# biodatageeks/polars-bio

Measured on AMD Instinct MI355X. Metric: overlap-pairs/sec, higher is better.
Workload: dtype int32; 1 GPU; overlap_100M_5M_24contig; probe_rows=100000000, build_rows=5000000, contigs=24, filter_op=Strict, parallelism=single GPU

## Files before the change

include/ivjoin.h:

```cpp
#ifndef IVJOIN_H
#define IVJOIN_H

#include <stdint.h>

#ifdef __cplusplus
extern "C" {
#endif

#define IVJ_OK            0
#define IVJ_EINVAL       -1
#define IVJ_EHIP         -2
#define IVJ_ENOMEM       -3
#define IVJ_ECAPACITY    -4
#define IVJ_ESTATE       -5
#define IVJ_EPEER        -6

#define IVJ_FILTER_WEAK   0
#define IVJ_FILTER_STRICT 1

#define IVJ_NEAREST_IGNORE_LEFT  1
#define IVJ_NEAREST_IGNORE_RIGHT 2

typedef struct ivj_ctx ivj_ctx;
typedef struct ivj_index ivj_index;
// ... 339 lines not shown
                                    const ivj_opts* opts, const char* suffix1, int64_t batch_rows, int64_t limit, void* out_stream);
int ivj_nearest_arrow_stream(ivj_ctx* ctx, void* df1_stream, void* df2_stream, const char* const* cols1, const char* const* cols2,
                             const ivj_opts* opts, const char* suffix1, const char* suffix2, int32_t with_distance, int64_t batch_rows,
                             int64_t limit, void* out_stream);

int ivj_overlap_arrow_stream_lazy(ivj_ctx* ctx, void* df1_stream, void* df2_stream, const char* const* cols1, const char* const* cols2,
                                  const ivj_opts* opts, const char* suffix1, const char* suffix2, int64_t batch_rows, int64_t max_batch_rows,
                                  int64_t limit, void* out_stream);
int ivj_count_overlaps_arrow_stream_lazy(ivj_ctx* ctx, void* df1_stream, void* df2_stream, const char* const* cols1, const char* const* cols2,
                                         const ivj_opts* opts, const char* suffix1, int64_t batch_rows, int64_t max_batch_rows, int64_t limit,
                                         void* out_stream);
int ivj_nearest_arrow_stream_lazy(ivj_ctx* ctx, void* df1_stream, void* df2_stream, const char* const* cols1, const char* const* cols2,
                                  const ivj_opts* opts, const char* suffix1, const char* suffix2, int32_t with_distance, int64_t batch_rows,
                                  int64_t max_batch_rows, int64_t limit, void* out_stream);

typedef struct {
    int64_t n1, n2;
    int32_t *contig1, *start1, *end1;
    int32_t *contig2, *start2, *end2;
    int32_t n_contigs;
    int64_t* name_offsets;
    char* name_bytes;
} ivj_arrow_keys;
int ivj_arrow_encode_keys(void* df1_stream, void* df2_stream, const char* const* cols1, const char* const* cols2, ivj_arrow_keys* out);
void ivj_arrow_keys_free(ivj_arrow_keys* keys);
int ivj_arrow_take_stream(void* in_stream, const int64_t* idx, int64_t n, int64_t batch_rows, void* out_stream);


int ivj_dev_alloc(ivj_ctx* ctx, int64_t bytes, void** out);
int ivj_dev_free(ivj_ctx* ctx, void* p);
int ivj_memcpy_h2d(ivj_ctx* ctx, void* dst_dev, const void* src_host, int64_t bytes);
int ivj_memcpy_d2h(ivj_ctx* ctx, void* dst_host, const void* src_dev, int64_t bytes);


int ivj_host_narrow_i32(const void* src, int32_t src_bytes, int32_t is_unsigned, int64_t n, int32_t* dst, int64_t* out_min, int64_t* out_max,
                        int32_t threads);

int ivj_host_encode_utf8(const void* offsets, int32_t offset_bytes, const uint8_t* data, const uint8_t* validity, int64_t validity_bit0, int64_t n,
                         int32_t* ids, int64_t* dict_rows, int32_t dict_cap, int32_t* n_values, int32_t threads);

int ivj_host_encode_keys64(const uint64_t* keys, int64_t n, int32_t* ids, int64_t* dict_rows, int32_t dict_cap, int32_t* n_values, int32_t threads);

int ivj_host_remap_i32(const void* idx, int32_t idx_bytes, int64_t n, const int32_t* remap, int64_t remap_len, int32_t* out, uint8_t* seen,
                       int32_t threads);

int ivj_host_take(const void* src, int32_t elem_bytes, int64_t n_src, const int32_t* idx, int64_t n, void* dst, int32_t threads);

int ivj_host_scatter(const void* src, int32_t row_bytes, int64_t n, const int32_t* idx, int64_t n_dst, void* dst, const int32_t* remap, int64_t remap_len,
                     int32_t threads);

int ivj_host_shard(const int32_t* contig, const int32_t* start, const int32_t* end, int64_t n, const int32_t* owner, int32_t n_contigs, int32_t world,
                   int64_t* counts, int32_t* const* out_contig, int32_t* const* out_start, int32_t* const* out_end, int32_t* const* out_row, int32_t threads);
int ivj_host_contig_hist(const int32_t* contig, int64_t n, int32_t n_contigs, int64_t* hist, int32_t threads);
int ivj_host_group_ids(const int32_t* probe_contig, const int32_t* const* probe_codes, int64_t n_probe, const int32_t* build_contig,
                       const int32_t* const* build_codes, int64_t n_build, int32_t n_cols, const int32_t* cards, int32_t n_contigs,
                       int32_t* probe_gid, int32_t* build_gid, int32_t* group_keys, int64_t keys_cap, int32_t* n_groups, int32_t threads);

int ivj_host_widen_i32(const int32_t* src, int64_t n, int64_t* dst, int32_t threads);

#ifdef __cplusplus
}
#endif
#endif
```

polars-bio_amd/csrc/host_index.hip.h:

```cpp
#pragma once

namespace {

int build_tables(ivj_ctx* ctx, ivj_index* ix);
bool cs_geom(int64_t n, int nc, int want_rows, CsGeom& g);
size_t cs_index_bytes(const CsGeom& g);
void cs_index_carve(ivj_index* ix, char* p);

int ensure_hier(ivj_ctx* ctx, ivj_index* ix) {
    if (ix->hier_built || ix->n <= 0) return IVJ_OK;
    const HierShape h = hier_shape(ix->n);
    const int64_t wgs = (((ix->n + 15) & ~(int64_t)15) + HIER_WG_ROWS - 1) / HIER_WG_ROWS;
    LAUNCH(ctx, "hier_low", k_hier_low, (unsigned)wgs, 256, (const int2*)ix->ep, ix->n, ix->hier, h);
    if (h.nlev >= 3) LAUNCH(ctx, "hier_high", k_hier_high, 1, 256, ix->hier, h, wgs);
    HIP_TRY(hipGetLastError());
    ix->hier_built = true;
    return IVJ_OK;
}

int need_tables(ivj_ctx* ctx, ivj_index* ix) {
    if (!ix->has_tables) return fail(IVJ_ESTATE, "this index was built for merge / cluster only (with_end_order & 2): it has no lookup tables");
    if (ix->tables_built) return IVJ_OK;
    return build_tables(ctx, ix);
}
// ... 216 lines not shown
    p.z_meta = align_up(sizeof(V3Meta)); p.z_st = align_up((size_t)V3_BUCKETS * 8); p.z_hs = align_up((size_t)p.hs_tiles * 8); p.z_tick = align_up(16);
    p.zero_bytes = p.z_meta + p.z_st + p.z_hs + p.z_tick;
    return p;
}
int index_sort_v3(ivj_ctx* ctx, ivj_index* ix, const ivj_side* build, const ivj_opts* opts, bool* done) {
    *done = false;
    const int64_t n = build->n;
    const int nc = opts->n_contigs;
    const int64_t tiles = (n + OS_TILE - 1) / OS_TILE;
    const V3Plan VP = v3_plan(n);
    const int64_t chunk = VP.chunk, hist_len = VP.hist_len, hs_tiles = VP.hs_tiles;
    const int nchunks = VP.nchunks;
    const size_t z_meta = VP.z_meta, z_st = VP.z_st, z_hs = VP.z_hs, zero_bytes = VP.zero_bytes;
    OsSort S;
    const size_t v2_bytes = os_sort_plan(S, n, nc);
    const bool own_z = ix->ix3_z == nullptr;
    IVJ_TRY(arena_reserve(ctx, std::max(v2_bytes, (own_z ? zero_bytes : 0) + align_up((size_t)hist_len * 4) + align_up((size_t)n * 16)) + 4096));
    char* z = own_z ? arena_take<char>(ctx, zero_bytes) : ix->ix3_z;
    uint32_t* hist = arena_take<uint32_t>(ctx, (size_t)hist_len);
    int4* recs = arena_take<int4>(ctx, (size_t)n);
    V3Meta* meta = (V3Meta*)z;
    unsigned long long* st_local = (unsigned long long*)(z + z_meta);
    unsigned long long* st_scan = (unsigned long long*)(z + z_meta + z_st);
    uint32_t* tick_scan = (uint32_t*)(z + z_meta + z_st + z_hs);
    if (own_z) HIP_TRY(hipMemsetAsync(z, 0, zero_bytes, ctx->stream));
    const size_t pass_lds = (size_t)v3_pass_lds().total;
    if (!ctx->ix3_attr_set) {
        HIP_TRY(hipFuncSetAttribute(reinterpret_cast<const void*>(&k_v3_scatter), hipFuncAttributeMaxDynamicSharedMemorySize, (int)pass_lds));
        HIP_TRY(hipFuncSetAttribute(reinterpret_cast<const void*>(&k_v3_local<true>), hipFuncAttributeMaxDynamicSharedMemorySize, 160 * 1024 - 256));
        HIP_TRY(hipFuncSetAttribute(reinterpret_cast<const void*>(&k_v3_local<false>), hipFuncAttributeMaxDynamicSharedMemorySize, 160 * 1024 - 256));
        ctx->ix3_attr_set = true;
    }
    const unsigned sgrid = (unsigned)(tiles < 512 ? tiles : 512);
    LAUNCH(ctx, "ix3_stats", k_v3_stats, sgrid, OS_THREADS, build->start, build->end, build->contig, n, nc, meta);
    LAUNCH(ctx, "ix3_hist", k_v3_hist, nchunks, OS_THREADS, build->contig, build->start, n, nc, meta, (int)chunk, nchunks, hist);
    LAUNCH(ctx, "ix_scan", (k_scan_lb_u32<SumOp, true>), hs_tiles, OS_THREADS, hist, hist_len, 0u, tick_scan, st_scan);
    const int ms_max = ctx->env_ix_merge >= 0 ? std::min(ctx->env_ix_merge, V3_MAX_MERGE) : V3_MAX_MERGE;
    const uint32_t hw_seq = ctx->hw ? ++ctx->hw_seq : 0u;
    LAUNCH(ctx, "ix3_check", k_v3_check, 1, OS_THREADS, (const uint32_t*)hist, nchunks, n, ms_max, meta, ctx->hw_dev, hw_seq);
    if (!ctx->hw) HIP_TRY(hipMemcpyAsync(ctx->h_total + 6, &meta->bad, 8, hipMemcpyDeviceToHost, ctx->stream));
    if (!ctx->ix3_event) HIP_TRY(hipEventCreateWithFlags(&ctx->ix3_event, hipEventDisableTiming));
    HIP_TRY(hipEventRecord(ctx->ix3_event, ctx->stream));
    t_begin(ctx, "ix3_pass");
    hipLaunchKernelGGL(k_v3_scatter, dim3((unsigned)nchunks), dim3(OS_THREADS), pass_lds, ctx->stream, build->contig, build->start, build->end, build->row_id,
                       recs, n, nc, meta, (int)chunk, nchunks, (const uint32_t*)hist);
    t_end(ctx);
    HIP_TRY(hipGetLastError());
    HIP_TRY(wait_event(ctx, ctx->ix3_event));
    uint32_t* hv = reinterpret_cast<uint32_t*>(ctx->h_total + 6);
    if (ctx->hw) {
        const volatile uint32_t* w = reinterpret_cast<volatile uint32_t*>(ctx->hw);
        if (w[2] == hw_seq) { hv[0] = w[0]; hv[1] = w[1]; }
        else {
            ++ctx->hw_misses;
            HIP_TRY(hipMemcpyAsync(ctx->h_total + 6, &meta->bad, 8, hipMemcpyDeviceToHost, ctx->stream));
            HIP_TRY(hipStreamSynchronize(ctx->stream));
        }
    }
    const uint32_t max_bucket = hv[1] & 0xffffffu;
    const int ms = (int)(hv[1] >> 24);
    if (hv[0] != 0u || max_bucket > (uint32_t)V3_CAP) { ++ctx->ix3_fallbacks; ++ctx->ix3_fallback_streak; ctx->ix3_builds_since_fallback = 0; return IVJ_OK; }
    ctx->ix3_fallback_streak = 0;
    const int cap = (int)std::max<uint32_t>(1024u, (max_bucket + 1023u) / 1024u * 1024u);
    const int bin_bits = cap <= 1024 ? 10 : (cap <= 2048 ? 11 : V3_MAX_BIN_BITS);
    const bool stage = ctx->env_ix_stage >= 0 ? ctx->env_ix_stage != 0 : cap <= 2048;
    const size_t local_lds = (size_t)v3_local_lds(cap, 1 << bin_bits, stage).total;
    with_bool(stage, [&](auto STAGE) {
        LAUNCH_LDS(ctx, "ix3_local", k_v3_local<STAGE>, V3_BUCKETS >> ms, OS_THREADS, local_lds, (const int4*)recs, (const uint32_t*)hist, nchunks, n, nc, cap, bin_bits, ms,
                   meta, st_local, ix->b_start, ix->ep, ix->b_row, ix->b_contig, ix->seg, ix->flags);
    });
    HIP_TRY(hipGetLastError());
    *done = true;
    return IVJ_OK;
}

int build_tables(ivj_ctx* ctx, ivj_index* ix) {
    const int nc = ix->n_contigs;
    const int64_t n = ix->n;
    if (n > 0 && nc > 0) {
        const int64_t lb_tiles = (ix->bins_len + LB_TILE - 1) / LB_TILE;
        const size_t zb = align_up((size_t)lb_tiles * 8) + align_up(16);
        IVJ_TRY(arena_reserve(ctx, zb + 4096));
        char* z = arena_take<char>(ctx, zb);
        HIP_TRY(hipMemsetAsync(z, 0, zb, ctx->stream));
        HIP_TRY(hipMemsetAsync(ix->bins, 0, (size_t)ix->bins_len * 4, ctx->stream));
        LAUNCH(ctx, "contig_meta", k_contig_meta, grid1d(nc, 256), 256, (const int32_t*)ix->seg, (const int32_t*)ix->b_start, nc, ix->cmeta);
        LAUNCH(ctx, "bins_mark", k_bins_mark, grid1d(n, 256), 256, (const int32_t*)ix->b_start, (const int32_t*)ix->b_contig, n, nc,
               (const int4*)ix->cmeta, ix->bins);
        LAUNCH(ctx, "bins_scan", (k_scan_lb_u32<MaxOp, false>), lb_tiles, OS_THREADS, ix->bins, ix->bins_len, 0u,
               (uint32_t*)(z + align_up((size_t)lb_tiles * 8)), (unsigned long long*)z);
        LAUNCH(ctx, "bins_records", k_bins_records, grid1d(ix->bins_len, 256), 256, (const uint32_t*)ix->bins, ix->bins_len,
// ... 95 lines not shown
```

polars-bio_amd/csrc/ivjoin.hip:

```cpp
#include "../../include/ivjoin.h"

#include <hip/hip_runtime.h>

#include <algorithm>
#include <atomic>
#include <chrono>
#include <cstdio>
#include <cstdlib>
#include <cstring>
#include <string>
#include <vector>
#include <thread>
#include <type_traits>

#include "probe.hip.h"
#include "slice.hip.h"
#include "cslice.hip.h"
#include "onesweep.hip.h"
#include "ixsort3.hip.h"
#include "scan.hip.h"
#include "group.hip.h"
#include "depth.hip.h"
#include "depth_sum.hip.h"
#include "depth_profile.hip.h"
// ... 1717 lines not shown
    *out = nullptr;
    if (bytes == 0) return IVJ_OK;
    hipError_t e = hipMalloc(out, (size_t)bytes);
    if (e != hipSuccess) return fail(IVJ_ENOMEM, std::string("hipMalloc: ") + hipGetErrorString(e));
    return IVJ_OK;
} IVJ_ABI_CATCH
int ivj_dev_free(ivj_ctx* ctx, void* p) try {
    if (!ctx) return fail(IVJ_EINVAL, "ctx is NULL");
    if (!p) return IVJ_OK;
    DeviceGuard g(ctx->device);
    HIP_TRY(hipStreamSynchronize(ctx->stream));
    HIP_TRY(hipFree(p));
    return IVJ_OK;
} IVJ_ABI_CATCH
int ivj_memcpy_h2d(ivj_ctx* ctx, void* dst_dev, const void* src_host, int64_t bytes) try {
    if (!ctx || bytes < 0) return fail(IVJ_EINVAL, "bad argument");
    if (bytes == 0) return IVJ_OK;
    DeviceGuard g(ctx->device);
    HostXfer copy(ctx->stream, &ctx->xfer);
    copy.h2d(dst_dev, src_host, (size_t)bytes);
    HIP_TRY(copy.finish());
    return IVJ_OK;
} IVJ_ABI_CATCH
int ivj_memcpy_d2h(ivj_ctx* ctx, void* dst_host, const void* src_dev, int64_t bytes) try {
    if (!ctx || bytes < 0) return fail(IVJ_EINVAL, "bad argument");
    if (bytes == 0) return IVJ_OK;
    DeviceGuard g(ctx->device);
    HostXfer copy(ctx->stream, &ctx->xfer);
    copy.d2h(dst_host, src_dev, (size_t)bytes);
    HIP_TRY(copy.finish());
    return IVJ_OK;
} IVJ_ABI_CATCH

}

#include "host_frontdoor.hip.h"
#include "host_arrow_stream.hip.h"
```

polars-bio_amd/csrc/ixsort3.hip.h:

```cpp
#pragma once
#include "onesweep.hip.h"

namespace ivj {

constexpr int V3_BUCKETS = OS_RADIX;
constexpr int V3_ITEMS = 4;
constexpr int V3_CAP = OS_THREADS * V3_ITEMS;
constexpr int V3_MAX_KEYS = 256;
constexpr int V3_MAX_BIN_BITS = 12;

struct V3Meta {
    uint32_t inverted;
    uint32_t pad0;
    uint32_t bad;
    uint32_t max_bucket;
    uint32_t ticket;
    uint32_t wbits;
    uint32_t pad[2];
    unsigned long long M;
    unsigned long long span;
    uint32_t cmax[V3_MAX_KEYS];
    uint32_t cimn[V3_MAX_KEYS];
    uint32_t base[V3_MAX_KEYS];
};

__device__ __forceinline__ uint32_t v3_bucket(uint32_t lin, unsigned long long M) { return (uint32_t)(((unsigned long long)lin * M) >> 32); }

__device__ __forceinline__ void v3_load_tables(const V3Meta* __restrict__ meta, int nk, uint32_t* l_base, uint32_t* l_cmin) {
    for (int k = threadIdx.x; k < nk; k += OS_THREADS) { l_base[k] = meta->base[k]; l_cmin[k] = ~meta->cimn[k]; }
}

__global__ __launch_bounds__(OS_THREADS) void k_v3_stats(const int32_t* __restrict__ start, const int32_t* __restrict__ end,
                                                        const int32_t* __restrict__ contig, int64_t n, int32_t n_contigs, V3Meta* __restrict__ meta) {
    __shared__ uint32_t l_mx[V3_MAX_KEYS], l_imn[V3_MAX_KEYS];
    __shared__ uint32_t l_inv;
    const int tid = threadIdx.x, nk = n_contigs + 1;
    for (int k = tid; k < V3_MAX_KEYS; k += OS_THREADS) { l_mx[k] = 0u; l_imn[k] = 0u; }
    if (tid == 0) l_inv = 0u;
    __syncthreads();
    uint32_t inv = 0;
    for (int64_t i = (int64_t)blockIdx.x * OS_THREADS + tid; i < n; i += (int64_t)gridDim.x * OS_THREADS) {
        const int32_t s = start[i], c0 = contig[i];
        const int c = (uint32_t)c0 < (uint32_t)n_contigs ? c0 : n_contigs;
        const uint32_t u = flip(s);
        if (u > l_mx[c]) atomicMax(&l_mx[c], u);
        if (~u > l_imn[c]) atomicMax(&l_imn[c], ~u);
        if (s > end[i] && c < n_contigs) inv = 1u;
    }
    if (inv) l_inv = 1u;
    __syncthreads();
    for (int k = tid; k < nk; k += OS_THREADS) {
        const uint32_t a = l_mx[k], b = l_imn[k];
        if (a > os_ld(&meta->cmax[k])) atomicMax(&meta->cmax[k], a);
        if (b > os_ld(&meta->cimn[k])) atomicMax(&meta->cimn[k], b);
    }
    if (tid == 0 && l_inv && !os_ld(&meta->inverted)) atomicOr(&meta->inverted, 1u);
}

struct V3Geom { unsigned long long M; uint32_t wbits; bool bad; };
__device__ __forceinline__ V3Geom v3_geometry(V3Meta* __restrict__ meta, int nk, uint32_t* l_base, uint32_t* l_cmin, unsigned long long* l_ws , bool record) {
    const int tid = threadIdx.x;
    unsigned long long sp = 0;
    uint32_t cmn = 0xffffffffu;
    if (tid < nk) {
        const uint32_t cmx = meta->cmax[tid], cim = meta->cimn[tid];
        cmn = ~cim;
        if ((cmx | cim) != 0u) sp = (unsigned long long)(cmx - cmn) + 1ull;
    }
    unsigned long long total;
    const unsigned long long pre = sl_block_exclusive_sum<unsigned long long>(sp, l_ws, &total);
    if (tid < nk) { l_base[tid] = (uint32_t)pre; l_cmin[tid] = cmn; if (record) meta->base[tid] = (uint32_t)pre; }
    if (tid == 0) {
        const bool bad = total == 0ull || total > 0xffffffffull;
        const unsigned long long M = bad ? 1ull : (1ull << 43) / total;
        const unsigned long long wmax = (1ull << 32) / M;
        const uint32_t wbits = (uint32_t)os_bits_for(wmax > 0xffffffffull ? 0xffffffffu : (uint32_t)wmax);
        l_ws[OS_WAVES] = M;
        l_ws[OS_WAVES + 1] = (unsigned long long)wbits | (bad ? (1ull << 32) : 0ull);
        if (record) { meta->bad = bad ? 1u : 0u; meta->span = total; meta->M = M; meta->wbits = wbits; }
    }
    __syncthreads();
    V3Geom g;
    g.M = l_ws[OS_WAVES];
    g.wbits = (uint32_t)l_ws[OS_WAVES + 1];
    g.bad = (l_ws[OS_WAVES + 1] >> 32) != 0ull;
    return g;
}

__global__ __launch_bounds__(OS_THREADS) void k_v3_hist(const int32_t* __restrict__ contig, const int32_t* __restrict__ start, int64_t n,
                                                       int32_t n_contigs, V3Meta* __restrict__ meta, int chunk, int nchunks,
                                                       uint32_t* __restrict__ hist) {
    __shared__ uint32_t h[V3_BUCKETS];
    __shared__ uint32_t l_base[V3_MAX_KEYS], l_cmin[V3_MAX_KEYS];
    __shared__ unsigned long long l_ws[OS_WAVES + 2];
    const V3Geom g = v3_geometry(meta, n_contigs + 1, l_base, l_cmin, l_ws, blockIdx.x == 0);
    if (g.bad) return;
    const unsigned long long M = g.M;
    for (int k = threadIdx.x; k < V3_BUCKETS; k += OS_THREADS) h[k] = 0;
    __syncthreads();
    const int64_t base = (int64_t)blockIdx.x * chunk;
    const int64_t end = base + chunk < n ? base + chunk : n;
    for (int64_t i = base + threadIdx.x; i < end; i += OS_THREADS) {
        const int32_t c0 = contig[i];
        const int c = (uint32_t)c0 < (uint32_t)n_contigs ? c0 : n_contigs;
        const uint32_t lin = l_base[c] + (flip(start[i]) - l_cmin[c]);
        atomicAdd(&h[v3_bucket(lin, M)], 1u);
    }
    __syncthreads();
    for (int k = threadIdx.x; k < V3_BUCKETS; k += OS_THREADS) hist[(int64_t)k * nchunks + blockIdx.x] = h[k];
}

constexpr int V3_MAX_MERGE = 5;
__global__ __launch_bounds__(OS_THREADS) void k_v3_check(const uint32_t* __restrict__ off, int nchunks, int64_t n, int ms_max, V3Meta* __restrict__ meta,
                                                        uint32_t* __restrict__ hw, uint32_t hw_seq) {
    __shared__ uint32_t wmx[V3_MAX_MERGE + 1][OS_WAVES];
    if (meta->bad) {
        if (threadIdx.x == 0 && hw) { hw_store(hw + 0, 1u); hw_store(hw + 1, 0u); hw_store(hw + 2, hw_seq); }
        return;
    }
    const int tid = threadIdx.x;
    uint32_t sz[2];
#pragma unroll
    for (int q = 0; q < 2; ++q) {
        const int b = 2 * tid + q;
        const uint32_t a = off[(int64_t)b * nchunks];
        const uint32_t z = b + 1 < V3_BUCKETS ? off[(int64_t)(b + 1) * nchunks] : (uint32_t)n;
        sz[q] = z - a;
    }
    uint32_t mx[V3_MAX_MERGE + 1];
    mx[0] = sz[0] > sz[1] ? sz[0] : sz[1];
    uint32_t sum = sz[0] + sz[1];
    mx[1] = sum;
#pragma unroll
    for (int k = 2; k <= V3_MAX_MERGE; ++k) { sum += __shfl_xor(sum, 1 << (k - 2), kWave); mx[k] = sum; }
#pragma unroll
    for (int k = 0; k <= V3_MAX_MERGE; ++k) {
#pragma unroll
        for (int d = kWave / 2; d > 0; d >>= 1) { const uint32_t o = __shfl_xor(mx[k], d, kWave); mx[k] = o > mx[k] ? o : mx[k]; }
        if ((tid & (kWave - 1)) == 0) wmx[k][tid / kWave] = mx[k];
    }
    __syncthreads();
    if (tid == 0) {
        uint32_t best = 0, best_ms = 0;
#pragma unroll
        for (int k = 0; k <= V3_MAX_MERGE; ++k) {
            uint32_t m = 0;
#pragma unroll
            for (int w = 0; w < OS_WAVES; ++w) m = wmx[k][w] > m ? wmx[k][w] : m;
            if (k == 0 || (k <= ms_max && m <= (uint32_t)V3_CAP)) { best = m; best_ms = (uint32_t)k; }
        }
        meta->max_bucket = best | (best_ms << 24);
        if (hw) { hw_store(hw + 0, 0u); hw_store(hw + 1, best | (best_ms << 24)); hw_store(hw + 2, hw_seq); }
    }
}

struct V3PassLds { OsPassLds P; int tbase, tcmin, total; };
__host__ __device__ inline V3PassLds v3_pass_lds() {
    V3PassLds L;
    L.P = os_pass_lds();
    int o = (L.P.total + 15) & ~15;
    L.tbase = o; o += 4 * V3_MAX_KEYS;
    L.tcmin = o; o += 4 * V3_MAX_KEYS;
    L.total = o;
    return L;
}

__global__ __launch_bounds__(OS_THREADS) void k_v3_scatter(const int32_t* __restrict__ contig, const int32_t* __restrict__ start,
                                                          const int32_t* __restrict__ end, const int32_t* __restrict__ row_id,
                                                          int4* __restrict__ dst, int64_t n, int32_t n_contigs, V3Meta* __restrict__ meta,
                                                          int chunk, int nchunks, const uint32_t* __restrict__ off ) {
    extern __shared__ __attribute__((aligned(16))) unsigned char os_lds[];
    const V3PassLds LL = v3_pass_lds();
    const OsPassLds& L = LL.P;
    int4* l_rec = reinterpret_cast<int4*>(os_lds + L.rec);
    unsigned short* wcnt = reinterpret_cast<unsigned short*>(os_lds + L.wcnt);
    unsigned short* l_d = reinterpret_cast<unsigned short*>(os_lds + L.d);
    uint32_t* base = reinterpret_cast<uint32_t*>(os_lds + L.base);
    uint32_t* lstart = reinterpret_cast<uint32_t*>(os_lds + L.lstart);
    uint32_t* wsum = reinterpret_cast<uint32_t*>(os_lds + L.wsum);
    uint32_t* l_base = reinterpret_cast<uint32_t*>(os_lds + LL.tbase);
    uint32_t* l_cmin = reinterpret_cast<uint32_t*>(os_lds + LL.tcmin);
    if (meta->bad) return;
    const unsigned long long M = meta->M;
    const int tid = threadIdx.x, w = tid / kWave, lane = tid & (kWave - 1);
    v3_load_tables(meta, n_contigs + 1, l_base, l_cmin);
    for (int k = tid; k < OS_RADIX; k += OS_THREADS) base[k] = off[(int64_t)k * nchunks + blockIdx.x];
    for (int k = tid; k < OS_RADIX * OS_WAVES / 2; k += OS_THREADS) reinterpret_cast<uint32_t*>(wcnt)[k] = 0;
    __syncthreads();
    const int64_t cbase = (int64_t)blockIdx.x * chunk;
    const int64_t cend = cbase + chunk < n ? cbase + chunk : n;
    const uint64_t lt = lanemask_lt();
    unsigned short* my = wcnt + w * OS_RADIX;
    const int el0 = w * (OS_ITEMS * kWave) + lane;
    int4 nxt[OS_ITEMS];
    auto load_tile = [&](int64_t tb) {
        const int tn = (int)((cend - tb) < (int64_t)OS_TILE ? (cend - tb) : (int64_t)OS_TILE);
#pragma unroll
        for (int j = 0; j < OS_ITEMS; ++j) {
            const int il = el0 + j * kWave;
            nxt[j] = il < tn ? os_load_record(true, contig, start, end, row_id, nullptr, tb + il, n_contigs) : make_int4(0, 0, 0, 0);
        }
    };
    if (cbase < cend) load_tile(cbase);
    for (int64_t tbase = cbase; tbase < cend; tbase += OS_TILE) {
        const int tile_n = (int)((cend - tbase) < (int64_t)OS_TILE ? (cend - tbase) : (int64_t)OS_TILE);
        int4 r[OS_ITEMS];
        uint32_t d[OS_ITEMS], rank[OS_ITEMS];
#pragma unroll
        for (int j = 0; j < OS_ITEMS; ++j) {
            r[j] = nxt[j];
            d[j] = v3_bucket(l_base[r[j].w] + (flip(r[j].x) - l_cmin[r[j].w]), M);
        }
        if (tbase + OS_TILE < cend) load_tile(tbase + OS_TILE);
#pragma unroll
        for (int j = 0; j < OS_ITEMS; ++j) {
            const bool valid = el0 + j * kWave < tile_n;
            uint64_t peers = __ballot(valid);
#pragma unroll
            for (int b = 0; b < OS_BITS; ++b) {
                const bool bit = (d[j] >> b) & 1u;
                const uint64_t m = __ballot(valid && bit);
// ... 265 lines not shown
```

polars-bio_amd/polars_bio_amd/_engine.py:

```python
from __future__ import annotations

import ctypes as C
import os
import threading
from typing import Optional, Tuple

import numpy as np

_HERE = os.path.dirname(os.path.abspath(__file__))
LIB_PATH = os.path.join(_HERE, "lib", "libivjoin_hip.so")

FILTER_WEAK = 0
FILTER_STRICT = 1

ABI_SYMBOLS = [
    "ivj_last_error", "ivj_version", "ivj_abi_version", "ivj_device_count", "ivj_host_mem_available", "ivj_ctx_create", "ivj_ctx_destroy",
    "ivj_ctx_set_stream", "ivj_ctx_sync", "ivj_ctx_enable_timing", "ivj_ctx_get_timings", "ivj_ctx_profile_mark",
    "ivj_overlap", "ivj_pairs_free", "ivj_count_overlaps", "ivj_nearest",
    "ivj_index_build_dev", "ivj_index_free", "ivj_overlap_count_dev", "ivj_overlap_fill_dev", "ivj_overlap_fused_dev",
    "ivj_count_overlaps_dev", "ivj_nearest_dev",
    "ivj_overlap_thresh", "ivj_count_overlaps_thresh", "ivj_overlap_thresh_dev", "ivj_count_overlaps_thresh_dev",
    "ivj_overlap_select", "ivj_rowsel_free", "ivj_overlap_select_dev", "ivj_overlap_outer",
    "ivj_side_from_arrow", "ivj_materialize_dev", "ivj_overlap_fused_rows_dev", "ivj_take_dev", "ivj_take", "ivj_overlap_rows", "ivj_rows_free", "ivj_rows_export_arrow",
    "ivj_subtract", "ivj_complement", "ivj_pieces_free", "ivj_subtract_dev",
    "ivj_merge", "ivj_merged_free", "ivj_cluster", "ivj_coverage", "ivj_cluster_dev", "ivj_merge_dev", "ivj_coverage_dev",
    "ivj_merge_agg", "ivj_merge_agg_free", "ivj_merge_agg_dev",
    "ivj_overlap_agg", "ivj_overlap_agg_dev", "ivj_permute_overlaps", "ivj_permute_overlaps_dev",
    "ivj_overlap_wagg", "ivj_overlap_wagg_dev", "ivj_signal_profile", "ivj_signal_profile_dev",
    "ivj_overlap_bases", "ivj_overlap_bases_dev", "ivj_depth_profile", "ivj_depth_profile_dev",
    "ivj_depth", "ivj_blocks_free", "ivj_depth_dev", "ivj_depth_summary", "ivj_depth_summary_dev",
    "ivj_setop", "ivj_regions_free", "ivj_set_stats", "ivj_setop_dev", "ivj_set_stats_dev",
    "ivj_multi_inter", "ivj_segments_free", "ivj_multi_inter_dev",
    "ivj_stream_open", "ivj_stream_submit", "ivj_stream_flush", "ivj_stream_set_nearest_ignore", "ivj_stream_close",
    "ivj_dev_alloc", "ivj_dev_free", "ivj_memcpy_h2d", "ivj_memcpy_d2h",
    "ivj_comm_unique_id", "ivj_comm_create", "ivj_comm_create_local", "ivj_comm_destroy", "ivj_comm_info",
    "ivj_allgather_counts", "ivj_allgatherv_dev", "ivj_overlap_allgather_dev",
    "ivj_count_overlaps_allgather_dev", "ivj_nearest_allgather_dev",
    "ivj_overlap_arrow_stream", "ivj_count_overlaps_arrow_stream", "ivj_nearest_arrow_stream", "ivj_arrow_encode_keys", "ivj_arrow_keys_free",
    "ivj_overlap_arrow_stream_lazy", "ivj_count_overlaps_arrow_stream_lazy", "ivj_nearest_arrow_stream_lazy",
    "ivj_arrow_take_stream",
    "ivj_host_shard", "ivj_host_contig_hist", "ivj_group_ids_dev", "ivj_host_group_ids",
    "ivj_host_narrow_i32", "ivj_host_encode_utf8", "ivj_host_encode_keys64", "ivj_host_remap_i32", "ivj_host_take", "ivj_host_scatter", "ivj_host_widen_i32",
]

ABI_VERSION = 6
STREAM_OVERLAP, STREAM_COUNT, STREAM_NEAREST = 0, 1, 2
NEAREST_IGNORE_LEFT, NEAREST_IGNORE_RIGHT = 1, 2
DEPTH_PROFILE_MAX_BINS = 4096

SETOP_INTERSECTION, SETOP_UNION, SETOP_DIFFERENCE, SETOP_SYMMETRIC_DIFFERENCE = 0, 1, 2, 3
SETOPS = {"intersection": SETOP_INTERSECTION, "union": SETOP_UNION, "difference": SETOP_DIFFERENCE,
          "symmetric_difference": SETOP_SYMMETRIC_DIFFERENCE}

MAX_FRAMES = 64
MULTI_SEGMENTS, MULTI_CONSENSUS = 0, 1

AGG_SUM, AGG_MIN, AGG_MAX, AGG_MEAN, AGG_COUNT = 1, 2, 4, 8, 16
AGG_OPS = {"sum": AGG_SUM, "min": AGG_MIN, "max": AGG_MAX, "mean": AGG_MEAN, "count": AGG_COUNT}
AGG_I64, AGG_F64 = 0, 1
MAX_AGG_COLS = 16

ROW_COLUMNS = ("probe_idx", "build_idx", "contig", "start_1", "end_1", "start_2", "end_2")


IVJ_ECAPACITY, IVJ_ESTATE, IVJ_EPEER = -4, -5, -6

SELECT_SEMI, SELECT_ANTI = 0, 1
# ... 191 lines not shown
        L.ivj_permute_overlaps.argtypes = [vp, P, P, O, vp, vp, C.c_int64, vp, vp]
        L.ivj_permute_overlaps_dev.argtypes = [vp, vp, P, O, vp, vp, C.c_int64, vp, vp]
        L.ivj_depth.argtypes = [vp, P, O, C.POINTER(_Blocks)]
        L.ivj_blocks_free.argtypes = [C.POINTER(_Blocks)]
        L.ivj_blocks_free.restype = None
        L.ivj_depth_dev.argtypes = [vp, vp, O, C.c_int64, vp, vp, vp, vp, C.POINTER(C.c_int64)]
        L.ivj_setop.argtypes = [vp, P, P, O, C.c_int32, C.POINTER(_Regions)]
        L.ivj_regions_free.argtypes = [C.POINTER(_Regions)]
        L.ivj_regions_free.restype = None
        L.ivj_set_stats.argtypes = [vp, P, P, O, C.POINTER(C.c_int64), C.POINTER(C.c_int64)]
        L.ivj_setop_dev.argtypes = [vp, vp, vp, O, C.c_int32, C.c_int64, vp, vp, vp, C.POINTER(C.c_int64)]
        L.ivj_set_stats_dev.argtypes = [vp, vp, vp, O, C.POINTER(C.c_int64), C.POINTER(C.c_int64)]
        L.ivj_multi_inter.argtypes = [vp, P, C.c_int32, O, C.c_int32, C.c_int32, C.POINTER(_Segments)]
        L.ivj_segments_free.argtypes = [C.POINTER(_Segments)]
        L.ivj_segments_free.restype = None
        L.ivj_multi_inter_dev.argtypes = [vp, C.POINTER(vp), C.c_int32, O, C.c_int32, C.c_int32, C.c_int64, vp, vp, vp, vp, C.POINTER(C.c_int64)]
        L.ivj_coverage_dev.argtypes = [vp, vp, P, O, vp]
        L.ivj_overlap_bases.argtypes = [vp, P, P, O, vp]
        L.ivj_overlap_bases_dev.argtypes = [vp, vp, P, O, vp]
        L.ivj_depth_profile.argtypes = [vp, P, vp, C.c_int32, P, O, vp]
        L.ivj_depth_profile_dev.argtypes = [vp, vp, P, vp, C.c_int32, O, vp]
        L.ivj_depth_summary.argtypes = [vp, P, P, O, vp, C.c_int32, vp, vp]
        L.ivj_depth_summary_dev.argtypes = [vp, vp, P, O, vp, C.c_int32, vp, vp]
        L.ivj_stream_open.argtypes = [vp, P, O, C.c_int, C.c_int64, C.POINTER(vp)]
        L.ivj_stream_submit.argtypes = [vp, P, C.POINTER(_StreamResult)]
        L.ivj_stream_flush.argtypes = [vp, C.POINTER(_StreamResult)]
        L.ivj_stream_set_nearest_ignore.argtypes = [vp, C.c_int32]
        L.ivj_stream_close.argtypes = [vp]
        L.ivj_stream_close.restype = None
        L.ivj_dev_alloc.argtypes = [vp, C.c_int64, C.POINTER(vp)]
        L.ivj_dev_free.argtypes = [vp, vp]
        L.ivj_memcpy_h2d.argtypes = [vp, vp, vp, C.c_int64]
        L.ivj_memcpy_d2h.argtypes = [vp, vp, vp, C.c_int64]
        L.ivj_comm_unique_id.argtypes = [vp]
        L.ivj_comm_create.argtypes = [vp, vp, C.c_int, C.c_int, C.POINTER(vp)]
        L.ivj_comm_create_local.argtypes = [C.POINTER(vp), C.c_int, C.POINTER(vp)]
        L.ivj_comm_destroy.argtypes = [vp]
        L.ivj_comm_destroy.restype = None
        L.ivj_comm_info.argtypes = [vp, C.POINTER(C.c_int), C.POINTER(C.c_int)]
        L.ivj_allgather_counts.argtypes = [vp, C.c_int64, C.POINTER(C.c_int64)]
        L.ivj_allgatherv_dev.argtypes = [vp, C.POINTER(vp), C.POINTER(vp), C.c_int, C.c_int, C.POINTER(C.c_int64)]
        L.ivj_overlap_allgather_dev.argtypes = [vp, vp, P, O, C.c_int, vp, vp, C.c_int64, C.POINTER(C.c_int64), C.POINTER(C.c_int64)]
        L.ivj_count_overlaps_allgather_dev.argtypes = [vp, vp, P, O, C.c_int64, vp]
        L.ivj_nearest_allgather_dev.argtypes = [vp, vp, P, O, C.c_int64, vp, vp, vp]
        L.ivj_host_narrow_i32.argtypes = [vp, C.c_int32, C.c_int32, C.c_int64, vp, C.POINTER(C.c_int64), C.POINTER(C.c_int64), C.c_int32]
        L.ivj_host_encode_utf8.argtypes = [vp, C.c_int32, vp, vp, C.c_int64, C.c_int64, vp, vp, C.c_int32, C.POINTER(C.c_int32), C.c_int32]
        L.ivj_host_encode_keys64.argtypes = [vp, C.c_int64, vp, vp, C.c_int32, C.POINTER(C.c_int32), C.c_int32]
        L.ivj_host_remap_i32.argtypes = [vp, C.c_int32, C.c_int64, vp, C.c_int64, vp, vp, C.c_int32]
        L.ivj_host_take.argtypes = [vp, C.c_int32, C.c_int64, vp, C.c_int64, vp, C.c_int32]
        L.ivj_host_scatter.argtypes = [vp, C.c_int32, C.c_int64, vp, C.c_int64, vp, vp, C.c_int64, C.c_int32]
        L.ivj_host_widen_i32.argtypes = [vp, C.c_int64, vp, C.c_int32]
        L.ivj_host_shard.argtypes = [vp, vp, vp, C.c_int64, vp, C.c_int32, C.c_int32, vp, vp, vp, vp, vp, C.c_int32]
        L.ivj_host_contig_hist.argtypes = [vp, C.c_int64, C.c_int32, vp, C.c_int32]
        L.ivj_group_ids_dev.argtypes = [vp, vp, C.POINTER(vp), C.c_int64, vp, C.POINTER(vp), C.c_int64, C.c_int32, vp, C.c_int32, vp, vp, vp,
                                        C.c_int64, C.POINTER(C.c_int32)]
        L.ivj_host_group_ids.argtypes = [vp, C.POINTER(vp), C.c_int64, vp, C.POINTER(vp), C.c_int64, C.c_int32, vp, C.c_int32, vp, vp, vp,
                                         C.c_int64, C.POINTER(C.c_int32), C.c_int32]
        names3 = C.POINTER(C.c_char_p)
        L.ivj_overlap_arrow_stream.argtypes = [vp, vp, vp, names3, names3, O, C.c_char_p, C.c_char_p, C.c_int64, C.c_int64, vp]
        L.ivj_count_overlaps_arrow_stream.argtypes = [vp, vp, vp, names3, names3, O, C.c_char_p, C.c_int64, C.c_int64, vp]
        L.ivj_nearest_arrow_stream.argtypes = [vp, vp, vp, names3, names3, O, C.c_char_p, C.c_char_p, C.c_int32, C.c_int64, C.c_int64, vp]
        L.ivj_overlap_arrow_stream_lazy.argtypes = [vp, vp, vp, names3, names3, O, C.c_char_p, C.c_char_p, C.c_int64, C.c_int64, C.c_int64, vp]
        L.ivj_count_overlaps_arrow_stream_lazy.argtypes = [vp, vp, vp, names3, names3, O, C.c_char_p, C.c_int64, C.c_int64, C.c_int64, vp]
        L.ivj_nearest_arrow_stream_lazy.argtypes = [vp, vp, vp, names3, names3, O, C.c_char_p, C.c_char_p, C.c_int32, C.c_int64, C.c_int64, C.c_int64, vp]
        L.ivj_arrow_encode_keys.argtypes = [vp, vp, names3, names3, C.POINTER(_ArrowKeys)]
        L.ivj_arrow_keys_free.argtypes = [C.POINTER(_ArrowKeys)]
# ... 970 lines not shown
            return
        rows = int(min(batch_rows, n))
        with self.probe_stream(build, strict, n_contigs, STREAM_OVERLAP, rows, copy=False) as st:
            def emit(res):
                lo = res["batch"] * rows
                return (res["probe_idx"] + np.int32(lo)), res["build_idx"].copy()
            for lo in range(0, n, rows):
                hi = min(lo + rows, n)
                res = st.submit((pc[lo:hi], ps[lo:hi], pe[lo:hi]))
                if res is not None:
                    yield emit(res)
            while True:
                res = st.flush()
                if res is None:
                    break
                yield emit(res)

    def dev_alloc(self, nbytes: int) -> int:
        p = C.c_void_p()
        _check(self.L, self.L.ivj_dev_alloc(self.h, nbytes, C.byref(p)), "ivj_dev_alloc")
        return p.value or 0

    def dev_free(self, ptr: int):
        _check(self.L, self.L.ivj_dev_free(self.h, C.c_void_p(ptr)), "ivj_dev_free")

    def h2d(self, dst_ptr: int, arr: np.ndarray):
        arr = np.ascontiguousarray(arr)
        _check(self.L, self.L.ivj_memcpy_h2d(self.h, C.c_void_p(dst_ptr), arr.ctypes.data, arr.nbytes), "ivj_memcpy_h2d")

    def d2h(self, arr: np.ndarray, src_ptr: int):
        assert arr.flags.c_contiguous
        _check(self.L, self.L.ivj_memcpy_d2h(self.h, arr.ctypes.data, C.c_void_p(src_ptr), arr.nbytes), "ivj_memcpy_d2h")


UNIQUE_ID_BYTES = 128


def comm_unique_id() -> bytes:
    L = load_library()
    buf = C.create_string_buffer(UNIQUE_ID_BYTES)
    _check(L, L.ivj_comm_unique_id(buf), "ivj_comm_unique_id")
    return buf.raw


class Comm:

    def __init__(self, engine: Engine, unique_id: Optional[bytes], rank: int, world: int, _handle=None):
        self.engine, self.rank, self.world = engine, rank, world
        self.L = load_library()
        if _handle is not None:
            self.h = _handle
            return
        h = C.c_void_p()
        idbuf = C.create_string_buffer(unique_id, UNIQUE_ID_BYTES) if unique_id is not None else None
        _check(self.L, self.L.ivj_comm_create(engine.h, idbuf, int(rank), int(world), C.byref(h)), "ivj_comm_create")
        self.h = h

    @staticmethod
    def create_local(engines):
        L = load_library()
        n = len(engines)
        ctxs = (C.c_void_p * n)(*[e.h for e in engines])
        out = (C.c_void_p * n)()
        _check(L, L.ivj_comm_create_local(ctxs, n, out), "ivj_comm_create_local")
        return [Comm(e, None, i, n, _handle=C.c_void_p(out[i])) for i, e in enumerate(engines)]

# ... 164 lines not shown
```

Baseline: 111.5 billion overlap-pairs/s.

## Fold bucket check into scatter kernel, spin on host word, vectorize stats

When a host-visible word is available, the bucket-size check moves into block 0 of the scatter kernel and writes one 64-bit value holding the result and a sequence number. The host then spin-waits on that word instead of waiting on an event recorded before the scatter launch. This removes a separate single-block kernel launch and lets the scatter kernel be queued before the host reads the check result. The stats kernel also gains an int4 vectorized load path when all three input arrays are 16-byte aligned. A debug export of index arrays is added as well. The risk is that the host now waits until the scatter kernel runs, and block 0 of that kernel does extra serial work.

```diff
diff --git a/include/ivjoin.h b/include/ivjoin.h
--- a/include/ivjoin.h
+++ b/include/ivjoin.h
@@ -395,6 +395,8 @@
 int ivj_memcpy_h2d(ivj_ctx* ctx, void* dst_dev, const void* src_host, int64_t bytes);
 int ivj_memcpy_d2h(ivj_ctx* ctx, void* dst_host, const void* src_dev, int64_t bytes);
 
+int ivj_index_debug_array(ivj_ctx* ctx, ivj_index* ix, int32_t which, void* dst_host, int64_t cap_bytes, int64_t* bytes);
+
 
 int ivj_host_narrow_i32(const void* src, int32_t src_bytes, int32_t is_unsigned, int64_t n, int32_t* dst, int64_t* out_min, int64_t* out_max,
                         int32_t threads);
diff --git a/polars-bio_amd/csrc/host_index.hip.h b/polars-bio_amd/csrc/host_index.hip.h
--- a/polars-bio_amd/csrc/host_index.hip.h
+++ b/polars-bio_amd/csrc/host_index.hip.h
@@ -272,31 +272,36 @@
         ctx->ix3_attr_set = true;
     }
     const unsigned sgrid = (unsigned)(tiles < 512 ? tiles : 512);
-    LAUNCH(ctx, "ix3_stats", k_v3_stats, sgrid, OS_THREADS, build->start, build->end, build->contig, n, nc, meta);
+    const int stats_vec = (((uintptr_t)build->start | (uintptr_t)build->end | (uintptr_t)build->contig) & 15u) == 0 ? 1 : 0;
+    LAUNCH(ctx, "ix3_stats", k_v3_stats, sgrid, OS_THREADS, build->start, build->end, build->contig, n, nc, stats_vec, meta);
     LAUNCH(ctx, "ix3_hist", k_v3_hist, nchunks, OS_THREADS, build->contig, build->start, n, nc, meta, (int)chunk, nchunks, hist);
     LAUNCH(ctx, "ix_scan", (k_scan_lb_u32<SumOp, true>), hs_tiles, OS_THREADS, hist, hist_len, 0u, tick_scan, st_scan);
     const int ms_max = ctx->env_ix_merge >= 0 ? std::min(ctx->env_ix_merge, V3_MAX_MERGE) : V3_MAX_MERGE;
     const uint32_t hw_seq = ctx->hw ? ++ctx->hw_seq : 0u;
-    LAUNCH(ctx, "ix3_check", k_v3_check, 1, OS_THREADS, (const uint32_t*)hist, nchunks, n, ms_max, meta, ctx->hw_dev, hw_seq);
-    if (!ctx->hw) HIP_TRY(hipMemcpyAsync(ctx->h_total + 6, &meta->bad, 8, hipMemcpyDeviceToHost, ctx->stream));
-    if (!ctx->ix3_event) HIP_TRY(hipEventCreateWithFlags(&ctx->ix3_event, hipEventDisableTiming));
-    HIP_TRY(hipEventRecord(ctx->ix3_event, ctx->stream));
+    if (!ctx->hw) {
+        LAUNCH(ctx, "ix3_check", k_v3_check, 1, OS_THREADS, (const uint32_t*)hist, nchunks, n, ms_max, meta);
+        HIP_TRY(hipMemcpyAsync(ctx->h_total + 6, &meta->bad, 8, hipMemcpyDeviceToHost, ctx->stream));
+        if (!ctx->ix3_event) HIP_TRY(hipEventCreateWithFlags(&ctx->ix3_event, hipEventDisableTiming));
+        HIP_TRY(hipEventRecord(ctx->ix3_event, ctx->stream));
+    }
     t_begin(ctx, "ix3_pass");
     hipLaunchKernelGGL(k_v3_scatter, dim3((unsigned)nchunks), dim3(OS_THREADS), pass_lds, ctx->stream, build->contig, build->start, build->end, build->row_id,
-                       recs, n, nc, meta, (int)chunk, nchunks, (const uint32_t*)hist);
+                       recs, n, nc, meta, (int)chunk, nchunks, (const uint32_t*)hist, ms_max, ctx->hw_dev, hw_seq);
     t_end(ctx);
     HIP_TRY(hipGetLastError());
-    HIP_TRY(wait_event(ctx, ctx->ix3_event));
     uint32_t* hv = reinterpret_cast<uint32_t*>(ctx->h_total + 6);
     if (ctx->hw) {
-        const volatile uint32_t* w = reinterpret_cast<volatile uint32_t*>(ctx->hw);
-        if (w[2] == hw_seq) { hv[0] = w[0]; hv[1] = w[1]; }
+        const volatile unsigned long long* w = reinterpret_cast<volatile unsigned long long*>(ctx->hw);
+        auto arrived = [&] { return (uint32_t)(w[0] >> 32) == hw_seq; };
+        hipError_t pe = hipSuccess;
+        if (!spin_wait(ctx, [&] { return arrived() ? hipSuccess : hipErrorNotReady; }, &pe)) HIP_TRY(hipStreamSynchronize(ctx->stream));
+        if (arrived()) { const uint32_t v = (uint32_t)w[0]; hv[0] = (v & V3_HW_BAD) ? 1u : 0u; hv[1] = v & ~V3_HW_BAD; }
         else {
             ++ctx->hw_misses;
             HIP_TRY(hipMemcpyAsync(ctx->h_total + 6, &meta->bad, 8, hipMemcpyDeviceToHost, ctx->stream));
             HIP_TRY(hipStreamSynchronize(ctx->stream));
         }
-    }
+    } else HIP_TRY(wait_event(ctx, ctx->ix3_event));
     const uint32_t max_bucket = hv[1] & 0xffffffu;
     const int ms = (int)(hv[1] >> 24);
     if (hv[0] != 0u || max_bucket > (uint32_t)V3_CAP) { ++ctx->ix3_fallbacks; ++ctx->ix3_fallback_streak; ctx->ix3_builds_since_fallback = 0; return IVJ_OK; }
diff --git a/polars-bio_amd/csrc/ivjoin.hip b/polars-bio_amd/csrc/ivjoin.hip
--- a/polars-bio_amd/csrc/ivjoin.hip
+++ b/polars-bio_amd/csrc/ivjoin.hip
@@ -1773,6 +1773,46 @@
     return IVJ_OK;
 } IVJ_ABI_CATCH
 
+int ivj_index_debug_array(ivj_ctx* ctx, ivj_index* ix, int32_t which, void* dst_host, int64_t cap_bytes, int64_t* bytes) try {
+    if (!ctx || !ix || !bytes || ix->ctx != ctx) return fail(IVJ_EINVAL, "bad argument");
+    DeviceGuard g(ctx->device);
+    HIP_TRY(hipStreamSynchronize(ctx->stream));
+    const CsGeom& G = ix->cs_g;
+    const size_t n = (size_t)ix->n, nc = (size_t)ix->n_contigs;
+    const int32_t geom[5] = {G.R, G.nb, G.n_contigs, G.cps, G.ncells};
+    const int64_t counters[2] = {(int64_t)ctx->ix3_fallbacks, (int64_t)ctx->hw_misses};
+    const void* src = nullptr;
+    size_t len = 0;
+    bool host = false;
+    if (which >= 6 && which <= 14 && !(ix->cs_ok && ix->cs_built)) return fail(IVJ_ESTATE, "the slice tables of this index are not built");
+    switch (which) {
+        case 0: src = ix->b_start; len = n * 4; break;
+        case 1: src = ix->ep; len = n * 8; break;
+        case 2: src = ix->b_row; len = n * 4; break;
+        case 3: src = ix->b_contig; len = n * 4; break;
+        case 4: src = ix->seg; len = (nc + 2) * 4; break;
+        case 5: src = ix->flags; len = 8; break;
+        case 6: src = ix->cs_bound; len = (size_t)(G.nb + 1) * 4; break;
+        case 7: src = ix->cs_spl; len = (size_t)G.nb * 8; break;
+        case 8: src = ix->cs_cm; len = nc * 16; break;
+        case 9: src = ix->cs_cell; len = (size_t)G.ncells * 4; break;
+        case 10: src = ix->cs_bins; len = (size_t)G.nb * (size_t)(2 * G.R + CS_BIN_STRIDE_PAD) * 2; break;
+        case 11: src = ix->cs_smeta; len = (size_t)G.nb * 32; break;
+        case 12: src = geom; len = sizeof(geom); host = true; break;
+        case 13: src = ctx->sl_gh; len = (size_t)(G.nb + 3) * 4; break;
+        case 14: src = ctx->sl_rstart; len = (size_t)(G.nb + 1) * 4; break;
+        case 15: src = counters; len = sizeof(counters); host = true; break;
+        default: return fail(IVJ_EINVAL, "unknown array");
+    }
+    *bytes = (int64_t)len;
+    if (!dst_host || len == 0) return IVJ_OK;
+    if (cap_bytes < (int64_t)len) return fail(IVJ_EINVAL, "destination too small");
+    if (!src) return fail(IVJ_ESTATE, "the array does not exist");
+    if (host) std::memcpy(dst_host, src, len);
+    else HIP_TRY(hipMemcpy(dst_host, src, len, hipMemcpyDeviceToHost));
+    return IVJ_OK;
+} IVJ_ABI_CATCH
+
 }
 
 #include "host_frontdoor.hip.h"
diff --git a/polars-bio_amd/csrc/ixsort3.hip.h b/polars-bio_amd/csrc/ixsort3.hip.h
--- a/polars-bio_amd/csrc/ixsort3.hip.h
+++ b/polars-bio_amd/csrc/ixsort3.hip.h
@@ -30,8 +30,21 @@
     for (int k = threadIdx.x; k < nk; k += OS_THREADS) { l_base[k] = meta->base[k]; l_cmin[k] = ~meta->cimn[k]; }
 }
 
+__device__ __forceinline__ void v3_stats_row(int32_t s, int32_t e, int32_t c0, int32_t n_contigs, uint32_t* l_mx, uint32_t* l_imn, uint32_t& inv) {
+    const int c = (uint32_t)c0 < (uint32_t)n_contigs ? c0 : n_contigs;
+    const uint32_t u = flip(s);
+    if (u > l_mx[c]) atomicMax(&l_mx[c], u);
+    if (~u > l_imn[c]) atomicMax(&l_imn[c], ~u);
+    if (s > e && c < n_contigs) inv = 1u;
+}
+__device__ __forceinline__ void v3_stats_row4(const int4 s, const int4 e, const int4 c, int32_t n_contigs, uint32_t* l_mx, uint32_t* l_imn, uint32_t& inv) {
+    v3_stats_row(s.x, e.x, c.x, n_contigs, l_mx, l_imn, inv);
+    v3_stats_row(s.y, e.y, c.y, n_contigs, l_mx, l_imn, inv);
+    v3_stats_row(s.z, e.z, c.z, n_contigs, l_mx, l_imn, inv);
+    v3_stats_row(s.w, e.w, c.w, n_contigs, l_mx, l_imn, inv);
+}
 __global__ __launch_bounds__(OS_THREADS) void k_v3_stats(const int32_t* __restrict__ start, const int32_t* __restrict__ end,
-                                                        const int32_t* __restrict__ contig, int64_t n, int32_t n_contigs, V3Meta* __restrict__ meta) {
+                                                        const int32_t* __restrict__ contig, int64_t n, int32_t n_contigs, int vec, V3Meta* __restrict__ meta) {
     __shared__ uint32_t l_mx[V3_MAX_KEYS], l_imn[V3_MAX_KEYS];
     __shared__ uint32_t l_inv;
     const int tid = threadIdx.x, nk = n_contigs + 1;
@@ -39,14 +52,24 @@
     if (tid == 0) l_inv = 0u;
     __syncthreads();
     uint32_t inv = 0;
-    for (int64_t i = (int64_t)blockIdx.x * OS_THREADS + tid; i < n; i += (int64_t)gridDim.x * OS_THREADS) {
-        const int32_t s = start[i], c0 = contig[i];
-        const int c = (uint32_t)c0 < (uint32_t)n_contigs ? c0 : n_contigs;
-        const uint32_t u = flip(s);
-        if (u > l_mx[c]) atomicMax(&l_mx[c], u);
-        if (~u > l_imn[c]) atomicMax(&l_imn[c], ~u);
-        if (s > end[i] && c < n_contigs) inv = 1u;
-    }
+    const int64_t gid = (int64_t)blockIdx.x * OS_THREADS + tid, stride = (int64_t)gridDim.x * OS_THREADS;
+    int64_t i0 = 0;
+    if (vec) {
+        const int64_t nv = n >> 2;
+        const int4* __restrict__ s4 = reinterpret_cast<const int4*>(start);
+        const int4* __restrict__ e4 = reinterpret_cast<const int4*>(end);
+        const int4* __restrict__ c4 = reinterpret_cast<const int4*>(contig);
+        int64_t i = gid;
+        for (; i + stride < nv; i += 2 * stride) {
+            const int4 sa = s4[i], ca = c4[i], ea = e4[i];
+            const int4 sb = s4[i + stride], cb = c4[i + stride], eb = e4[i + stride];
+            v3_stats_row4(sa, ea, ca, n_contigs, l_mx, l_imn, inv);
+            v3_stats_row4(sb, eb, cb, n_contigs, l_mx, l_imn, inv);
+        }
+        if (i < nv) v3_stats_row4(s4[i], e4[i], c4[i], n_contigs, l_mx, l_imn, inv);
+        i0 = nv << 2;
+    }
+    for (int64_t i = i0 + gid; i < n; i += stride) v3_stats_row(start[i], end[i], contig[i], n_contigs, l_mx, l_imn, inv);
     if (inv) l_inv = 1u;
     __syncthreads();
     for (int k = tid; k < nk; k += OS_THREADS) {
@@ -111,20 +134,20 @@
 }
 
 constexpr int V3_MAX_MERGE = 5;
-__global__ __launch_bounds__(OS_THREADS) void k_v3_check(const uint32_t* __restrict__ off, int nchunks, int64_t n, int ms_max, V3Meta* __restrict__ meta,
-                                                        uint32_t* __restrict__ hw, uint32_t hw_seq) {
-    __shared__ uint32_t wmx[V3_MAX_MERGE + 1][OS_WAVES];
-    if (meta->bad) {
-        if (threadIdx.x == 0 && hw) { hw_store(hw + 0, 1u); hw_store(hw + 1, 0u); hw_store(hw + 2, hw_seq); }
-        return;
-    }
+constexpr uint32_t V3_HW_BAD = 1u << 31;
+__device__ __forceinline__ void v3_hw_store(uint32_t* hw, uint32_t v, uint32_t hw_seq) {
+    __hip_atomic_store(reinterpret_cast<unsigned long long*>(hw), (unsigned long long)v | ((unsigned long long)hw_seq << 32), __ATOMIC_RELAXED, __HIP_MEMORY_SCOPE_SYSTEM);
+}
+template <class BucketStart>
+__device__ __forceinline__ void v3_check_body(BucketStart&& bstart, int64_t n, int ms_max, V3Meta* __restrict__ meta, uint32_t* __restrict__ hw, uint32_t hw_seq,
+                                              uint32_t (*wmx)[OS_WAVES]) {
     const int tid = threadIdx.x;
     uint32_t sz[2];
 #pragma unroll
     for (int q = 0; q < 2; ++q) {
         const int b = 2 * tid + q;
-        const uint32_t a = off[(int64_t)b * nchunks];
-        const uint32_t z = b + 1 < V3_BUCKETS ? off[(int64_t)(b + 1) * nchunks] : (uint32_t)n;
+        const uint32_t a = bstart(b);
+        const uint32_t z = b + 1 < V3_BUCKETS ? bstart(b + 1) : (uint32_t)n;
         sz[q] = z - a;
     }
     uint32_t mx[V3_MAX_MERGE + 1];
@@ -150,8 +173,13 @@
             if (k == 0 || (k <= ms_max && m <= (uint32_t)V3_CAP)) { best = m; best_ms = (uint32_t)k; }
         }
         meta->max_bucket = best | (best_ms << 24);
-        if (hw) { hw_store(hw + 0, 0u); hw_store(hw + 1, best | (best_ms << 24)); hw_store(hw + 2, hw_seq); }
-    }
+        if (hw) v3_hw_store(hw, best | (best_ms << 24), hw_seq);
+    }
+}
+__global__ __launch_bounds__(OS_THREADS) void k_v3_check(const uint32_t* __restrict__ off, int nchunks, int64_t n, int ms_max, V3Meta* __restrict__ meta) {
+    __shared__ uint32_t wmx[V3_MAX_MERGE + 1][OS_WAVES];
+    if (meta->bad) return;
+    v3_check_body([&](int b) { return off[(int64_t)b * nchunks]; }, n, ms_max, meta, nullptr, 0u, wmx);
 }
 
 struct V3PassLds { OsPassLds P; int tbase, tcmin, total; };
@@ -168,7 +196,8 @@
 __global__ __launch_bounds__(OS_THREADS) void k_v3_scatter(const int32_t* __restrict__ contig, const int32_t* __restrict__ start,
                                                           const int32_t* __restrict__ end, const int32_t* __restrict__ row_id,
                                                           int4* __restrict__ dst, int64_t n, int32_t n_contigs, V3Meta* __restrict__ meta,
-                                                          int chunk, int nchunks, const uint32_t* __restrict__ off ) {
+                                                          int chunk, int nchunks, const uint32_t* __restrict__ off ,
+                                                          int ms_max, uint32_t* __restrict__ hw , uint32_t hw_seq) {
     extern __shared__ __attribute__((aligned(16))) unsigned char os_lds[];
     const V3PassLds LL = v3_pass_lds();
     const OsPassLds& L = LL.P;
@@ -180,13 +209,20 @@
     uint32_t* wsum = reinterpret_cast<uint32_t*>(os_lds + L.wsum);
     uint32_t* l_base = reinterpret_cast<uint32_t*>(os_lds + LL.tbase);
     uint32_t* l_cmin = reinterpret_cast<uint32_t*>(os_lds + LL.tcmin);
-    if (meta->bad) return;
+    if (meta->bad) {
+        if (hw && blockIdx.x == 0 && threadIdx.x == 0) v3_hw_store(hw, V3_HW_BAD, hw_seq);
+        return;
+    }
     const unsigned long long M = meta->M;
     const int tid = threadIdx.x, w = tid / kWave, lane = tid & (kWave - 1);
     v3_load_tables(meta, n_contigs + 1, l_base, l_cmin);
     for (int k = tid; k < OS_RADIX; k += OS_THREADS) base[k] = off[(int64_t)k * nchunks + blockIdx.x];
     for (int k = tid; k < OS_RADIX * OS_WAVES / 2; k += OS_THREADS) reinterpret_cast<uint32_t*>(wcnt)[k] = 0;
     __syncthreads();
+    if (hw && blockIdx.x == 0) {
+        v3_check_body([&](int b) { return base[b]; }, n, ms_max, meta, hw, hw_seq, reinterpret_cast<uint32_t (*)[OS_WAVES]>(l_rec));
+        __syncthreads();
+    }
     const int64_t cbase = (int64_t)blockIdx.x * chunk;
     const int64_t cend = cbase + chunk < n ? cbase + chunk : n;
     const uint64_t lt = lanemask_lt();
diff --git a/polars-bio_amd/polars_bio_amd/_engine.py b/polars-bio_amd/polars_bio_amd/_engine.py
--- a/polars-bio_amd/polars_bio_amd/_engine.py
+++ b/polars-bio_amd/polars_bio_amd/_engine.py
@@ -32,7 +32,7 @@
     "ivj_setop", "ivj_regions_free", "ivj_set_stats", "ivj_setop_dev", "ivj_set_stats_dev",
     "ivj_multi_inter", "ivj_segments_free", "ivj_multi_inter_dev",
     "ivj_stream_open", "ivj_stream_submit", "ivj_stream_flush", "ivj_stream_set_nearest_ignore", "ivj_stream_close",
-    "ivj_dev_alloc", "ivj_dev_free", "ivj_memcpy_h2d", "ivj_memcpy_d2h",
+    "ivj_dev_alloc", "ivj_dev_free", "ivj_memcpy_h2d", "ivj_memcpy_d2h", "ivj_index_debug_array",
     "ivj_comm_unique_id", "ivj_comm_create", "ivj_comm_create_local", "ivj_comm_destroy", "ivj_comm_info",
     "ivj_allgather_counts", "ivj_allgatherv_dev", "ivj_overlap_allgather_dev",
     "ivj_count_overlaps_allgather_dev", "ivj_nearest_allgather_dev",
@@ -290,6 +290,7 @@
         L.ivj_dev_free.argtypes = [vp, vp]
         L.ivj_memcpy_h2d.argtypes = [vp, vp, vp, C.c_int64]
         L.ivj_memcpy_d2h.argtypes = [vp, vp, vp, C.c_int64]
+        L.ivj_index_debug_array.argtypes = [vp, vp, C.c_int32, vp, C.c_int64, C.POINTER(C.c_int64)]
         L.ivj_comm_unique_id.argtypes = [vp]
         L.ivj_comm_create.argtypes = [vp, vp, C.c_int, C.c_int, C.POINTER(vp)]
         L.ivj_comm_create_local.argtypes = [C.POINTER(vp), C.c_int, C.POINTER(vp)]
@@ -1326,6 +1327,14 @@
         assert arr.flags.c_contiguous
         _check(self.L, self.L.ivj_memcpy_d2h(self.h, arr.ctypes.data, C.c_void_p(src_ptr), arr.nbytes), "ivj_memcpy_d2h")
 
+    def index_debug_array(self, ix: DeviceIndex, which: int, dtype) -> np.ndarray:
+        nb = C.c_int64()
+        _check(self.L, self.L.ivj_index_debug_array(self.h, ix.handle, which, None, 0, C.byref(nb)), "ivj_index_debug_array")
+        out = np.empty(nb.value // np.dtype(dtype).itemsize, dtype)
+        if out.nbytes:
+            _check(self.L, self.L.ivj_index_debug_array(self.h, ix.handle, which, out.ctypes.data, out.nbytes, C.byref(nb)), "ivj_index_debug_array")
+        return out
+
 
 UNIQUE_ID_BYTES = 128
 
```

New measurement: 113.4 billion overlap-pairs/s, median of 6. 1.7% higher.
